# deepaksatna/Distributed-LLM-Training-Benchmark-Framework

Hardware: AMD Instinct MI355X
Metric: tokens_per_sec (higher is better)
Workload: dtype bf16

## Files before the change

### csrc/attention.hip

```cpp
#include <cstdlib>

#ifndef DLTB_ATTN_LPT
#define DLTB_ATTN_LPT 1
#endif
#ifndef DLTB_FWD_KS64
#define DLTB_FWD_KS64 4
#endif
#ifndef DLTB_CAUSAL_KS_CAP
#define DLTB_CAUSAL_KS_CAP 1
#endif
#ifndef DLTB_DQ_KS64
#define DLTB_DQ_KS64 3
#endif
#include "attn_mask.h"
#include "common.h"
#include "mfma_tiles.h"

namespace {

constexpr float kLog2e = 1.4426950408889634f;
constexpr int kBlockRows = 128;
constexpr int kTile = 64;

struct AttnArgs {
// ... 220 lines not shown
}
template <int D>
constexpr int fwd_stage_bytes() { return 2 * kTile * D * 2 + 1024; }
template <int D, int KS = fwd_ks<D>()>
constexpr int fwd_smem_bytes() { return fwd_nst<D, KS>() * KS * fwd_stage_bytes<D>(); }

template <int D, bool CAUSAL, bool DROP, int KS, bool WIN = false, bool DOC = false, bool QR = false>
__global__ __launch_bounds__(256 * KS) void attn_fwd_kernel(AttnArgs P) {
  static_assert(CAUSAL || !WIN, "a window is a band under the causal diagonal");
  static_assert((CAUSAL && !DROP) || !QR, "a query range is causal and without dropout (the packed mask is square)");
  static_assert((CAUSAL && !WIN) || !DOC, "document bounds are causal and carry the window themselves");
  constexpr bool BAND = WIN || DOC;
  constexpr int TB = kTile * D * 2;
  constexpr int NACC = D / 32;
  extern __shared__ __attribute__((aligned(16))) char smem[];
  const int tid = threadIdx.x, lane = tid & 63, w = tid >> 6, r = lane & 31, h = lane >> 5;
  const int qw = w & 3, sp = w >> 2, stid = tid & 255;
  const int T = P.T, nT = T / kTile;
  const int Tq = QR ? P.q_rows : T, qoff = QR ? P.q_begin : 0;
  int qb, bh;
  block_coords(Tq / kBlockRows, P.B * P.Hq, CAUSAL, qb, bh);
  if (QR) qb += qoff / kBlockRows;
  const int b = bh / P.Hq, hq = bh % P.Hq, hk = hq / (P.Hq / P.Hkv);
  const int q0 = qb * kBlockRows + qw * 32;
  const int qi = q0 + r;
  DLTB_DCHECK(qi < T && bh < P.B * P.Hq && hk < P.Hkv);

  bfx8 qf[D / 16];
  {
    const bf16_t* qrow = P.q + ((long)b * Tq + qi - qoff) * P.q_stride + hq * D;
#pragma unroll
    for (int s = 0; s < D / 16; ++s)
      qf[s] = scale_frag(__builtin_bit_cast(bfx8, ld16<uint4>(qrow + 16 * s + 8 * h)), P.scale * kLog2e);
  }
  const int nt = CAUSAL ? min(nT, (qb * kBlockRows + kBlockRows - 1) / kTile + 1) : nT;
  const int W = WIN ? P.window : 0;
  const int lo_q = DOC ? P.bounds[(long)b * T + qi] : 0;
  const int lo_w0 = DOC ? __builtin_amdgcn_readfirstlane(lo_q) : 0;
  const int lo_w1 = DOC ? __builtin_amdgcn_readlane(lo_q, 31) : 0;
  const int t_lo = WIN   ? max(0, qb * kBlockRows - W + 1) / kTile
                   : DOC ? min(max(P.bounds[(long)b * T + qb * kBlockRows], 0), qb * kBlockRows) / kTile
                         : 0;
  const int nit = (nt - t_lo + KS - 1) / KS;
  const bf16_t* kbase = P.k + (long)b * T * P.k_stride + hk * D;
  const bf16_t* vbase = P.v + (long)b * T * P.v_stride + hk * D;
  const uint32_t* mbase = DROP ? P.mask + (long)bh * nT * 2 * T : nullptr;
  const uint32_t* mrow = DROP ? mbase + (long)h * T + qi : nullptr;

  constexpr int NST = fwd_nst<D, KS>();
  constexpr int SB = fwd_stage_bytes<D>();
  constexpr int GL = 2 * GldsTile<D, kTile>::NI + (DROP ? 1 : 0);
  const int wv = __builtin_amdgcn_readfirstlane(qw);
  const int spu = __builtin_amdgcn_readfirstlane(sp);
  auto stage_ptr = [&](int it) { return smem + ((it % NST) * KS + spu) * SB; };
  uint32_t koff[GldsTile<D, kTile>::NI], voff[GldsTile<D, kTile>::NI];
  GldsTile<D, kTile>::offsets(P.k_stride, wv, lane, koff);
  GldsTile<D, kTile>::offsets(P.v_stride, wv, lane, voff);
  const uint32_t moff = (uint32_t)(mrow - mbase) * 4u;
  auto issue = [&](int it) {
    const int t = t_lo + it * KS + spu;
    if (it >= nit || t >= nt) return;
    char* st = smem + ((it % NST) * KS + spu) * SB;
    GldsTile<D, kTile>::load_sv(kbase + (long)t * kTile * P.k_stride, koff, st, wv);
    GldsTile<D, kTile>::load_sv(vbase + (long)t * kTile * P.v_stride, voff, st + TB, wv);
    if (DROP) glds4_sv(mbase + (long)t * 2 * T, moff, st + 2 * TB + wv * 256);
  };
  uint32_t kfo[D / 16], vfo[NACC][2];
#pragma unroll
  for (int s = 0; s < D / 16; ++s) kfo[s] = row_lane_off<D>(r, 2 * s + h);
#pragma unroll
  for (int dt = 0; dt < NACC; ++dt)
#pragma unroll
    for (int hf = 0; hf < 2; ++hf) vfo[dt][hf] = tr_lane_off<D>(dt * 32, hf, lane);
  wait_vm<0>();
#pragma unroll
  for (int i = 0; i < NST - 1; ++i) issue(i);

  f32x16 oacc[NACC];
#pragma unroll
  for (int dt = 0; dt < NACC; ++dt) oacc[dt] = f32x16{};
  float m = -INFINITY, l = 0.f;
  f32x16 mv = f32x16{};
  bool fresh = true;

  f32x16 sacc[2];
  auto s_tile = [&](const char* kt, int kv0) {
    const uint32_t kb = __builtin_amdgcn_readfirstlane(lds_addr(kt));
    uint32_t ka[D / 16];
#pragma unroll
    for (int s = 0; s < D / 16; ++s) ka[s] = lane_addr(kb, kfo[s]);
    sacc[0] = mfma32(row_frag_at<0>(ka[0]), qf[0], mv);
    sacc[1] = mfma32(row_frag_at<32 * D * 2>(ka[0]), qf[0], mv);
    static_for<D / 16 - 1>([&](auto S1) {
      constexpr int s = S1 + 1;
      sacc[0] = mfma32(row_frag_at<0>(ka[s]), qf[s], sacc[0]);
      sacc[1] = mfma32(row_frag_at<32 * D * 2>(ka[s]), qf[s], sacc[1]);
    });
    if (CAUSAL && kv0 + kTile - 1 > q0) {
#pragma unroll
      for (int n = 0; n < 2; ++n)
#pragma unroll
        for (int i = 0; i < 16; ++i)
          if (kv0 + 32 * n + (i & 3) + 8 * (i >> 2) + 4 * h > qi) sacc[n][i] = -INFINITY;
    }
    if (WIN && kv0 <= q0 + 31 - W) {
#pragma unroll
      for (int n = 0; n < 2; ++n)
#pragma unroll
        for (int i = 0; i < 16; ++i)
          if (kv0 + 32 * n + (i & 3) + 8 * (i >> 2) + 4 * h <= qi - W) sacc[n][i] = -INFINITY;
    }
    if (DOC && kv0 < lo_w1) {
#pragma unroll
      for (int n = 0; n < 2; ++n)
#pragma unroll
        for (int i = 0; i < 16; ++i)
          if (kv0 + 32 * n + (i & 3) + 8 * (i >> 2) + 4 * h < lo_q) sacc[n][i] = -INFINITY;
    }
  };
  auto row_max = [&]() {
    float mx = sacc[0][0];
#pragma unroll
    for (int n = 0; n < 2; ++n)
#pragma unroll
      for (int i = (n == 0 ? 1 : 0); i < 16; ++i) mx = fmaxf(mx, sacc[n][i]);
    const auto sw = __builtin_amdgcn_permlane32_swap(__float_as_uint(mx), __float_as_uint(mx), false, false);
    return fmaxf(__uint_as_float(sw[0]), __uint_as_float(sw[1]));
  };
  auto rescale = [&](float mx) {
    const float d = fresh ? mx : fmaxf(mx, 0.f);
    if (!fresh) {
      const float alpha = __builtin_amdgcn_exp2f(-d);
      l *= alpha;
#pragma unroll
      for (int dt = 0; dt < NACC; ++dt) oacc[dt] *= alpha;
    }
    m = fresh ? mx : m + d;
#pragma unroll
    for (int n = 0; n < 2; ++n) sacc[n] -= d;
    mv = splat16(-m);
    fresh = false;
  };
  auto rescale_win = [&](float mx) {
    const bool empty = m == -INFINITY;
    const bool moves = empty ? mx > -INFINITY : mx > kRescaleLog2;
    const float d = moves ? mx : 0.f;
    const float alpha = empty ? 1.f : __builtin_amdgcn_exp2f(-d);
    l *= alpha;
#pragma unroll
    for (int dt = 0; dt < NACC; ++dt) oacc[dt] *= alpha;
    m = moves ? (empty ? mx : m + d) : m;
#pragma unroll
    for (int n = 0; n < 2; ++n) sacc[n] -= d;
    mv = splat16(m == -INFINITY ? 0.f : -m);
  };
  auto softmax = [&]() {
    {
      const float mx = row_max();
      if constexpr (BAND) {
        if (__ballot(m == -INFINITY ? mx > -INFINITY : mx > kRescaleLog2)) rescale_win(mx);
      } else {
        if (fresh || __ballot(mx > kRescaleLog2)) rescale(mx);
      }
    }
    float ls0 = 0.f, ls1 = 0.f;
    static_for<32>([&](auto J) {
      constexpr int n = J / 16, i = J % 16;
      const float p = __builtin_amdgcn_exp2f(sacc[n][i]);
      if constexpr (i & 1) ls1 += p;
      else ls0 += p;
      sacc[n][i] = p;
    });
    l += ls0 + ls1;
  };
  auto pv = [&](const char* vt, uint32_t mw) {
    const uint32_t vb = __builtin_amdgcn_readfirstlane(lds_addr(vt));
    uint32_t va[NACC][2];
#pragma unroll
    for (int dt = 0; dt < NACC; ++dt)
#pragma unroll
      for (int hf = 0; hf < 2; ++hf) va[dt][hf] = lane_addr(vb, vfo[dt][hf]);
    static_for<4>([&](auto J) {
      constexpr int n = J / 2, s2 = J % 2;
      const bfx8 pf = pack_frag_keep<n, s2, DROP>(sacc[n], mw);
#pragma unroll
      for (int dt = 0; dt < NACC; ++dt)
        oacc[dt] = mfma32(tr_frag_at<(32 * n + 16 * s2) * D * 2>(va[dt][0], va[dt][1]), pf, oacc[dt]);
    });
  };
  auto mask_word = [&](const char* st) {
    return DROP ? *reinterpret_cast<const uint32_t*>(st + 2 * TB + wv * 256 + lane * 4) : 0u;
  };
  auto visible = [&](int t) {
    return t < nt && (!CAUSAL || t * kTile <= q0 + 31) && (!WIN || t * kTile + kTile - 1 > q0 - W) &&
           (!DOC || t * kTile + kTile - 1 >= lo_w0);
  };

  {
    for (int it = 0; it < nit; ++it) {
      const int t = t_lo + it * KS + spu;
      static_assert(NST <= 4, "the counted wait below assumes at most two later stages in flight");
      const int later = NST < 3 ? 0 : min(NST - 2, min(nit - 1, (nt - t_lo - 1 - spu) / KS) - it);
      if (NST > 3 && later >= 2) wait_vm<(NST > 3 ? 2 * GL : 0)>();
      else if (NST > 2 && later >= 1) wait_vm<(NST > 2 ? GL : 0)>();
      else wait_vm<0>();
      __builtin_amdgcn_s_barrier();
      issue(it + NST - 1);
      const char* kt = stage_ptr(it);
      if (visible(t)) {
        const uint32_t mw = mask_word(kt);
        s_tile(kt, t * kTile);
        softmax();
        pv(kt + TB, mw);
      }
    }
  }
  __syncthreads();
  if constexpr (KS > 1) {
    constexpr int NF = 16 * NACC + 2;
    static_assert((KS - 1) * 4 * NF * 64 * 4 <= NST * KS * SB, "merge buffer exceeds the LDS ring");
    float* red0 = reinterpret_cast<float*>(smem) + qw * NF * 64 + lane;
    if (sp > 0) {
      float* red = red0 + (sp - 1) * 4 * NF * 64;
      red[0] = m;
      red[64] = l;
#pragma unroll
      for (int dt = 0; dt < NACC; ++dt)
#pragma unroll
        for (int i = 0; i < 16; ++i) red[(2 + 16 * dt + i) * 64] = oacc[dt][i];
    }
    __syncthreads();
    if (sp > 0) return;
#pragma unroll
    for (int o = 0; o < KS - 1; ++o) {
      const float* red = red0 + o * 4 * NF * 64;
      const float m1 = red[0], l1 = red[64];
      const float mn = fmaxf(m, m1);
      const float a0 = BAND && m == -INFINITY ? 0.f : __builtin_amdgcn_exp2f(m - mn);
      const float a1 = BAND && m1 == -INFINITY ? 0.f : __builtin_amdgcn_exp2f(m1 - mn);
      m = mn;
      l = l * a0 + l1 * a1;
#pragma unroll
      for (int dt = 0; dt < NACC; ++dt)
#pragma unroll
        for (int i = 0; i < 16; ++i) oacc[dt][i] = oacc[dt][i] * a0 + red[(2 + 16 * dt + i) * 64] * a1;
    }
  }
  l += __shfl_xor(l, 32, 64);
  const float inv = (DROP ? P.drop_scale : 1.f) / l;
  bf16_t* orow = P.out + ((long)b * Tq + qi - qoff) * P.out_stride + hq * D;
  store_acc_rows<D>(orow, oacc, inv, h);
  if (h == 0) P.lse[((long)b * P.Hq + hq) * Tq + qi - qoff] = (m + __log2f(l)) * 0.69314718055994531f;
}



template <int D>
__global__ __launch_bounds__(256) void attn_bwd_delta_kernel(AttnArgs P) {
  constexpr int CH = D / 8;
  const long gid = blockIdx.x * (long)blockDim.x + threadIdx.x;
  const long row = gid / CH;
// ... 384 lines not shown
    const bf16_t* dorow = P.dout + ((long)b * Tq + qi - qoff) * P.do_stride + hq * D;
#pragma unroll
    for (int s = 0; s < D / 16; ++s) {
      qf[s] = __builtin_bit_cast(bfx8, ld16<uint4>(qrow + 16 * s + 8 * h));
      of[s] = __builtin_bit_cast(bfx8, ld16<uint4>(dorow + 16 * s + 8 * h));
    }
  }
  float dlt;
  if (P.o) {
    const bf16_t* orow = P.o + ((long)b * Tq + qi - qoff) * P.o_stride + hq * D;
    constexpr int NS = D / 16;
    float cs[NS];
#pragma unroll
    for (int s = 0; s < NS; ++s) {
      float a[8], c[8];
      unpack8(ld16<uint4>(orow + 16 * s + 8 * h), a);
      unpack8(__builtin_bit_cast(uint4, of[s]), c);
      float acc = 0.f;
#pragma unroll
      for (int e = 0; e < 8; ++e) acc += c[e] * a[e];
      cs[s] = acc;
    }
#pragma unroll
    for (int off = NS / 2; off > 0; off >>= 1)
#pragma unroll
      for (int s = 0; s < off; ++s) cs[s] += cs[s + off];
    dlt = cs[0] + __shfl_xor(cs[0], 32, 64);
    if (sp == 0 && h == 0) const_cast<float*>(P.delta)[bq * Tq + qi - qoff] = dlt;
  } else {
    dlt = P.delta[bq * Tq + qi - qoff];
  }
  const f32x16 nlv = splat16(-P.lse[bq * Tq + qi - qoff] * kLog2e);
  const float nd = -dlt * (DROP ? 1.f / P.drop_scale : 1.f);
  const f32x16 ndv = splat16(nd);
#pragma unroll
  for (int s = 0; s < D / 16; ++s) qf[s] = scale_frag(qf[s], P.scale * kLog2e);
  const uint32_t* mbase = DROP ? P.mask + (long)bq * nT * 2 * T : nullptr;
  const uint32_t* mrow = DROP ? mbase + (long)h * T + qi : nullptr;
  const int nt = CAUSAL ? min(nT, (qb * kBlockRows + kBlockRows - 1) / kTile + 1) : nT;
  const int W = WIN ? P.window : 0;
  const int lo_q = DOC ? P.bounds[(long)b * T + qi] : 0;
  const int lo_w0 = DOC ? __builtin_amdgcn_readfirstlane(lo_q) : 0;
  const int lo_w1 = DOC ? __builtin_amdgcn_readlane(lo_q, 31) : 0;
  const int t_lo = WIN   ? max(0, qb * kBlockRows - W + 1) / kTile
                   : DOC ? min(max(P.bounds[(long)b * T + qb * kBlockRows], 0), qb * kBlockRows) / kTile
                         : 0;
  const int nit = (nt - t_lo + KS - 1) / KS;
  const bf16_t* kbase = P.k + (long)b * T * P.k_stride + hk * D;
  const bf16_t* vbase = P.v + (long)b * T * P.v_stride + hk * D;

  constexpr int NST = dq_nst<D>();
  constexpr int SB = dq_stage_bytes<D>();
  constexpr int GL = 2 * GldsTile<D, kTile>::NI + (DROP ? 1 : 0);
  const int wv = __builtin_amdgcn_readfirstlane(qw);
  auto stage_ptr = [&](int it) { return smem + ((it % NST) * KS + sp) * SB; };
  uint32_t koff[GldsTile<D, kTile>::NI], voff[GldsTile<D, kTile>::NI];
  GldsTile<D, kTile>::offsets(P.k_stride, wv, lane, koff);
  GldsTile<D, kTile>::offsets(P.v_stride, wv, lane, voff);
  const uint32_t moff = (uint32_t)(mrow - mbase) * 4u;
  const int spu = __builtin_amdgcn_readfirstlane(sp);
  auto issue = [&](int it) {
    const int t = t_lo + it * KS + spu;
    if (it >= nit || t >= nt) return;
    char* st = smem + ((it % NST) * KS + spu) * SB;
    GldsTile<D, kTile>::load_sv(kbase + (long)t * kTile * P.k_stride, koff, st, wv);
    GldsTile<D, kTile>::load_sv(vbase + (long)t * kTile * P.v_stride, voff, st + TB, wv);
    if (DROP) glds4_sv(mbase + (long)t * 2 * T, moff, st + 2 * TB + wv * 256);
  };
  wait_vm<0>();
#pragma unroll
  for (int i = 0; i < NST - 1; ++i) issue(i);

  constexpr bool EMU2 = DOC && D == 128 && DROP && KS == 1;
  f32x16 dq[NACC], dq_odd[EMU2 ? NACC : 1];
#pragma unroll
  for (int dt = 0; dt < NACC; ++dt) dq[dt] = f32x16{};
  if constexpr (EMU2) {
#pragma unroll
    for (int dt = 0; dt < NACC; ++dt) dq_odd[dt] = f32x16{};
  }

  for (int it = 0; it < nit; ++it) {
    const int t = t_lo + it * KS + sp;
    static_assert(NST <= 3, "the counted wait below assumes at most one later stage in flight");
    if (NST > 2 && it + 1 < nit && t_lo + (it + 1) * KS + sp < nt) wait_vm<(NST > 2 ? GL : 0)>();
    else wait_vm<0>();
    __builtin_amdgcn_s_barrier();
    issue(it + NST - 1);
    const char* kt = stage_ptr(it);
    const char* vt = kt + TB;
    const uint32_t mw = DROP ? *reinterpret_cast<const uint32_t*>(kt + 2 * TB + wv * 256 + lane * 4) : 0u;
    const int kv0 = t * kTile;
    auto sdp = [&](int n, f32x16& sa, f32x16& dp) {
      sa = nlv;
      dp = ndv;
#pragma unroll
      for (int s = 0; s < D / 16; ++s) {
        sa = mfma32(row_frag<D>(kt, 32 * n + r, 2 * s + h), qf[s], sa);
        dp = mfma32(row_frag<D>(vt, 32 * n + r, 2 * s + h), of[s], dp);
      }
    };
    auto fin = [&](int n, const f32x16& sa, const f32x16& dp, auto ODD) {
      const bool diag = CAUSAL && kv0 + 32 * n + 31 > q0;
      const bool ledge = WIN && kv0 + 32 * n <= q0 + 31 - W;
      const bool dedge = DOC && kv0 + 32 * n < lo_w1;
      f32x16 ds;
      static_for<16>([&](auto I) {
        constexpr int i = I;
        float p = __builtin_amdgcn_exp2f(sa[i]);
        if (diag && kv0 + 32 * n + (i & 3) + 8 * (i >> 2) + 4 * h > qi) p = 0.f;
        if (ledge && kv0 + 32 * n + (i & 3) + 8 * (i >> 2) + 4 * h <= qi - W) p = 0.f;
        if (dedge && kv0 + 32 * n + (i & 3) + 8 * (i >> 2) + 4 * h < lo_q) p = 0.f;
        const float dpv = DROP ? (n == 0 ? keep_sel<mask_bit(0, i)>(dp[i], nd, mw)
                                         : keep_sel<mask_bit(1, i)>(dp[i], nd, mw)) : dp[i];
        ds[i] = p * dpv;
      });
#pragma unroll
      for (int s2 = 0; s2 < 2; ++s2) {
        const bfx8 sf = pack_frag<D>(ds, s2);
#pragma unroll
        for (int dt = 0; dt < NACC; ++dt)
          if constexpr (EMU2 && ODD) dq_odd[dt] = mfma32(tr_frag<D>(kt, 32 * n + 16 * s2, dt * 32, lane), sf, dq_odd[dt]);
          else dq[dt] = mfma32(tr_frag<D>(kt, 32 * n + 16 * s2, dt * 32, lane), sf, dq[dt]);
      }
    };
    if (t < nt) {
      {
#pragma unroll
        for (int n = 0; n < 2; ++n) {
          if (CAUSAL && kv0 + 32 * n > q0 + 31) continue;
          if (WIN && kv0 + 32 * n + 31 <= q0 - W) continue;
          if (DOC && kv0 + 32 * n + 31 < lo_w0) continue;
          f32x16 sa, dp;
          sdp(n, sa, dp);
          if (EMU2 && (it & 1)) fin(n, sa, dp, IC<1>{});
          else fin(n, sa, dp, IC<0>{});
        }
      }
    }
  }
  if constexpr (EMU2) {
#pragma unroll
    for (int dt = 0; dt < NACC; ++dt)
#pragma unroll
      for (int i = 0; i < 16; ++i) dq[dt][i] += dq_odd[dt][i];
  }
  __syncthreads();
  if constexpr (KS > 1) {
    constexpr int NF = 16 * NACC;
    static_assert((KS - 1) * 4 * NF * 64 * 4 <= dq_smem_bytes<D, KS>(), "merge buffer exceeds the LDS ring");
    float* red0 = reinterpret_cast<float*>(smem) + qw * NF * 64 + lane;
    if (sp > 0) {
      float* red = red0 + (sp - 1) * 4 * NF * 64;
#pragma unroll
      for (int dt = 0; dt < NACC; ++dt)
#pragma unroll
        for (int i = 0; i < 16; ++i) red[(16 * dt + i) * 64] = dq[dt][i];
    }
    __syncthreads();
    if (sp > 0) return;
#pragma unroll
    for (int o = 0; o < KS - 1; ++o)
#pragma unroll
      for (int dt = 0; dt < NACC; ++dt)
#pragma unroll
        for (int i = 0; i < 16; ++i) dq[dt][i] += red0[o * 4 * NF * 64 + (16 * dt + i) * 64];
  }
  bf16_t* dqrow = P.out + ((long)b * Tq + qi - qoff) * P.out_stride + hq * D;
  store_acc_rows<D>(dqrow, dq, P.scale * (DROP ? P.drop_scale : 1.f), h);
}

AttnArgs make_args(const void* q, const void* k, const void* v, long qs, long ks, long vs, int B,
                   int T, int Hq, int Hkv, float scale, int causal, uint32_t thr16,
                   float drop_scale, const int64_t* seed, int64_t site) {
  AttnArgs a{};
  a.q = (const bf16_t*)q;
  a.k = (const bf16_t*)k;
  a.v = (const bf16_t*)v;
  a.q_stride = qs;
  a.k_stride = ks;
  a.v_stride = vs;
  a.B = B;
  a.T = T;
  a.Hq = Hq;
  a.Hkv = Hkv;
  a.scale = scale;
  a.causal = causal;
  a.thr16 = thr16;
  a.drop_scale = drop_scale;
// ... 40 lines not shown
}

template <int D, bool C, bool DR, bool WIN = false, bool DOC = false, bool QR = false>
void launch_fwd(const AttnArgs& a, hipStream_t st) {
  constexpr int KS = fwd_ks<D, C>();
  constexpr int smem = fwd_smem_bytes<D, KS>();
  dim3 grid(((QR ? a.q_rows : a.T) / kBlockRows) * a.B * a.Hq);
  hipLaunchKernelGGL((attn_fwd_kernel<D, C, DR, KS, WIN, DOC, QR>), grid, dim3(256 * KS), smem, st, a);
}

#define DLTB_ATTN_DISPATCH(FN, D, C, DR, ...)           \
  do {                                                  \
    if (D == 64) {                                      \
      if (C) { if (DR) FN<64, true, true>(__VA_ARGS__); else FN<64, true, false>(__VA_ARGS__); } \
      else   { if (DR) FN<64, false, true>(__VA_ARGS__); else FN<64, false, false>(__VA_ARGS__); } \
    } else {                                            \
      if (C) { if (DR) FN<128, true, true>(__VA_ARGS__); else FN<128, true, false>(__VA_ARGS__); } \
      else   { if (DR) FN<128, false, true>(__VA_ARGS__); else FN<128, false, false>(__VA_ARGS__); } \
    }                                                   \
  } while (0)

#define DLTB_ATTN_DISPATCH_WIN(FN, D, DR, ...)          \
  do {                                                  \
    if (D == 64) { if (DR) FN<64, true, true, true>(__VA_ARGS__); else FN<64, true, false, true>(__VA_ARGS__); } \
    else         { if (DR) FN<128, true, true, true>(__VA_ARGS__); else FN<128, true, false, true>(__VA_ARGS__); } \
  } while (0)

#define DLTB_ATTN_DISPATCH_DOC(FN, D, DR, ...)          \
  do {                                                  \
    if (D == 64) { if (DR) FN<64, true, true, false, true>(__VA_ARGS__); else FN<64, true, false, false, true>(__VA_ARGS__); } \
    else         { if (DR) FN<128, true, true, false, true>(__VA_ARGS__); else FN<128, true, false, false, true>(__VA_ARGS__); } \
  } while (0)

#define DLTB_ATTN_DISPATCH_QR(FN, D, WIN, DOC, ...)     \
  do {                                                  \
    if (D == 64) {                                      \
      if (DOC) FN<64, true, false, false, true, true>(__VA_ARGS__);         \
      else if (WIN) FN<64, true, false, true, false, true>(__VA_ARGS__);    \
      else FN<64, true, false, false, false, true>(__VA_ARGS__);            \
    } else {                                            \
      if (DOC) FN<128, true, false, false, true, true>(__VA_ARGS__);        \
      else if (WIN) FN<128, true, false, true, false, true>(__VA_ARGS__);   \
      else FN<128, true, false, false, false, true>(__VA_ARGS__);           \
    }                                                   \
  } while (0)

bool windowed(int causal, int window, int T) { return causal && window > 0 && window < T; }

bool ranged(int q_begin, int q_end, int T) { return q_end > 0 && !(q_begin == 0 && q_end == T); }

}

void dltb_attn_init_attributes() {
  static bool done = false;
  if (done) return;
  done = true;
  set_attrs<64, false, false>();
  set_attrs<64, false, true>();
  set_attrs<64, true, false>();
  set_attrs<64, true, true>();
  set_attrs<128, false, false>();
  set_attrs<128, false, true>();
  set_attrs<128, true, false>();
  set_attrs<128, true, true>();
  set_attrs<64, true, false, true>();
  set_attrs<64, true, true, true>();
  set_attrs<128, true, false, true>();
  set_attrs<128, true, true, true>();
  set_attrs<64, true, false, false, true>();
  set_attrs<64, true, true, false, true>();
  set_attrs<128, true, false, false, true>();
  set_attrs<128, true, true, false, true>();
  set_attrs_qr<64, false, false>();
  set_attrs_qr<64, true, false>();
  set_attrs_qr<64, false, true>();
  set_attrs_qr<128, false, false>();
  set_attrs_qr<128, true, false>();
  set_attrs_qr<128, false, true>();
}

void dltb_attn_doc_bounds(const int64_t* idx, int* bounds, int B, int T, int64_t eos, int window, hipStream_t st) {
  hipLaunchKernelGGL(attn_doc_bounds_kernel, dim3(B), dim3(256), 0, st, idx, bounds, B, T, eos,
                     window > 0 && window < T ? window : 0);
}

void dltb_attn_mask(uint32_t* mask, int B, int T, int Hq, uint32_t thr16, const int64_t* seed,
                    int64_t site, hipStream_t st) {
  const dim3 grid(cdiv(T, 256), (unsigned)(B * Hq * (T / kTile) * 2));
  hipLaunchKernelGGL(attn_mask_kernel, grid, dim3(256), 0, st, mask, T, thr16, seed, site);
}

void dltb_attn_fwd(const void* q, const void* k, const void* v, void* o, float* lse,
                   const uint32_t* mask, long qs, long ks, long vs, long os, int B, int T, int Hq,
                   int Hkv, int D, float scale, int causal, uint32_t thr16, float drop_scale,
                   hipStream_t st, int window, const int* bounds, int q_begin, int q_end) {
  AttnArgs a = make_args(q, k, v, qs, ks, vs, B, T, Hq, Hkv, scale, causal, thr16, drop_scale,
                         nullptr, 0);
  a.out = (bf16_t*)o;
  a.out_stride = os;
  a.lse = lse;
  a.mask = mask;
  if (ranged(q_begin, q_end, T)) {
    a.q_begin = q_begin;
    a.q_rows = q_end - q_begin;
    a.bounds = bounds;
    a.window = windowed(causal, window, T) ? window : 0;
    DLTB_ATTN_DISPATCH_QR(launch_fwd, D, a.window != 0, bounds != nullptr, a, st);
    return;
  }
// ... 132 lines not shown
```

### csrc/gemm_tn.hip

```cpp
#include "common.h"
#include "launchers.h"
#include "mfma_tiles.h"

namespace {

constexpr int kTM = 256, kTN = 256;
constexpr int kRowB = 512;

struct TnArgs {
  const bf16_t* a;
  const bf16_t* b;
  bf16_t* c;
  long lda, ldb, ldc;
  long sa, sb, sc;
  int M, N, K, batch;
  int accumulate;
};

typedef __attribute__((ext_vector_type(4))) float f4;

DLTB_DEV f4 mfma16(bfx8 a, bfx8 b, f4 c) {
#if DLTB_F16
  return __builtin_amdgcn_mfma_f32_16x16x32_f16(a, b, c, 0, 0, 0);
#else
// ... 136 lines not shown
    o.y = pack_bf2(v[2], v[3]);
    *reinterpret_cast<uint2*>(cbase + (long)(16 * i) * g.ldc + 16 * j) = o;
  };
  if (g.accumulate) {
    uint2 old[8][4];
#pragma unroll
    for (int i = 0; i < 8; ++i)
#pragma unroll
      for (int j = 0; j < 4; ++j) old[i][j] = *reinterpret_cast<const uint2*>(cbase + (long)(16 * i) * g.ldc + 16 * j);
#pragma unroll
    for (int i = 0; i < 8; ++i)
#pragma unroll
      for (int j = 0; j < 4; ++j) {
        const float v[4] = {acc[i][j][0] + lo_bf(old[i][j].x), acc[i][j][1] + hi_bf(old[i][j].x),
                            acc[i][j][2] + lo_bf(old[i][j].y), acc[i][j][3] + hi_bf(old[i][j].y)};
        store(i, j, v);
      }
  } else {
#pragma unroll
    for (int i = 0; i < 8; ++i)
#pragma unroll
      for (int j = 0; j < 4; ++j) {
        const float v[4] = {acc[i][j][0], acc[i][j][1], acc[i][j][2], acc[i][j][3]};
        store(i, j, v);
      }
  }
}

}

bool dltb_gemm_tn_supported(int M, int N, int K) {
  return M > 0 && N > 0 && K > 0 && M % kTM == 0 && N % kTN == 0 && K % (2 * kTK3) == 0 && K / kTK3 >= 4;
}

int dltb_gemm_tn(const void* a, const void* b, void* c, long lda, long ldb, long ldc, long sa, long sb, long sc,
                 int M, int N, int K, int batch, int accumulate, hipStream_t st) {
  if (!dltb_gemm_tn_supported(M, N, K) || batch < 1) return -1;
  TnArgs g{};
  g.a = (const bf16_t*)a;
  g.b = (const bf16_t*)b;
  g.c = (bf16_t*)c;
  g.lda = lda;
  g.ldb = ldb;
  g.ldc = ldc;
  g.sa = sa;
  g.sb = sb;
  g.sc = sc;
  g.M = M;
  g.N = N;
  g.K = K;
  g.batch = batch;
  g.accumulate = accumulate;
  constexpr int smem = kRing3 * kStage3;
  static bool attr = false;
  if (!attr) {
    (void)hipFuncSetAttribute((const void*)gemm_tn_kernel, hipFuncAttributeMaxDynamicSharedMemorySize, smem);
    attr = true;
  }
  const dim3 grid((unsigned)((long)(M / kTM) * (N / kTN) * batch));
  hipLaunchKernelGGL(gemm_tn_kernel, grid, dim3(512), smem, st, g);
  return 0;
}
```

### csrc/mfma_tiles.h

```cpp
#pragma once
#include "common.h"

namespace {

typedef h16_t bfx8 __attribute__((ext_vector_type(8)));
typedef short s16x4 __attribute__((ext_vector_type(4)));
typedef __attribute__((address_space(3))) s16x4 lds_s16x4;

DLTB_DEV f32x16 mfma32(bfx8 a, bfx8 b, f32x16 c) {
#if DLTB_F16
  return __builtin_amdgcn_mfma_f32_32x32x16_f16(a, b, c, 0, 0, 0);
#else
  return __builtin_amdgcn_mfma_f32_32x32x16_bf16(a, b, c, 0, 0, 0);
#endif
}

template <int D>
DLTB_DEV int swz(int row) {
  if constexpr (D == 32) return (row >> 2) & 3;
  if constexpr (D == 64) return (((row >> 1) & 1) << 2) | ((row >> 2) & 3);
  else return ((row & 3) << 2) | ((row >> 2) & 3);
}
template <int D>
DLTB_DEV int toff(int row, int ch) {
  return row * (D * 2) + ((ch ^ swz<D>(row)) << 4);
}

template <int D>
DLTB_DEV bfx8 row_frag(const char* tile, int row, int ch) {
  uint4 v = *reinterpret_cast<const uint4*>(tile + toff<D>(row, ch));
  return __builtin_bit_cast(bfx8, v);
}

template <int D>
DLTB_DEV bfx8 tr_frag(const char* tile, int row_base, int col_base, int lane) {
  const int g = lane >> 4, i = lane & 15;
  const int row = row_base + 4 * (g >> 1) + (i >> 2);
  const int col = col_base + 16 * (g & 1) + 4 * (i & 3);
  const char* p0 = tile + toff<D>(row, col >> 3) + (col & 7) * 2;
  const char* p1 = tile + toff<D>(row + 8, col >> 3) + (col & 7) * 2;
  s16x4 a = __builtin_amdgcn_ds_read_tr16_b64_v4i16((lds_s16x4*)p0);
  s16x4 b = __builtin_amdgcn_ds_read_tr16_b64_v4i16((lds_s16x4*)p1);
  typedef short s16x8 __attribute__((ext_vector_type(8)));
  s16x8 c = {a[0], a[1], a[2], a[3], b[0], b[1], b[2], b[3]};
  return __builtin_bit_cast(bfx8, c);
}

template <int D>
DLTB_DEV uint32_t row_lane_off(int lane_row, int ch) { return (uint32_t)toff<D>(lane_row, ch); }
template <int D>
DLTB_DEV uint32_t tr_lane_off(int col_base, int half, int lane) {
  const int g = lane >> 4, i = lane & 15;
  const int row = 4 * (g >> 1) + (i >> 2) + 8 * half;
  const int col = col_base + 16 * (g & 1) + 4 * (i & 3);
  return (uint32_t)(toff<D>(row, col >> 3) + (col & 7) * 2);
}
typedef __attribute__((address_space(3))) const char lds_cchar;
typedef __attribute__((address_space(3))) const uint4 lds_u4;
DLTB_DEV uint32_t lds_addr(const void* p) { return (uint32_t)(size_t)(lds_cchar*)p; }
DLTB_DEV uint32_t lane_addr(uint32_t sbase, uint32_t off) {
  uint32_t a;
  asm("v_add_u32 %0, %1, %2" : "=v"(a) : "s"(sbase), "v"(off));
  return a;
}
template <int OFF>
DLTB_DEV bfx8 row_frag_at(uint32_t a) { return __builtin_bit_cast(bfx8, *(lds_u4*)(size_t)(a + OFF)); }
template <int OFF>
DLTB_DEV bfx8 tr_frag_at(uint32_t a0, uint32_t a1) {
  s16x4 a = __builtin_amdgcn_ds_read_tr16_b64_v4i16((lds_s16x4*)(size_t)(a0 + OFF));
  s16x4 b = __builtin_amdgcn_ds_read_tr16_b64_v4i16((lds_s16x4*)(size_t)(a1 + OFF));
  typedef short s16x8 __attribute__((ext_vector_type(8)));
  s16x8 c = {a[0], a[1], a[2], a[3], b[0], b[1], b[2], b[3]};
  return __builtin_bit_cast(bfx8, c);
}

DLTB_DEV void glds16_asm(const void* gsrc, const void* lds_dst) {
  const uint32_t lds = __builtin_amdgcn_readfirstlane(
      (uint32_t)(uintptr_t)(const __attribute__((address_space(3))) char*)lds_dst);
  uint32_t keep;
  asm volatile("s_mov_b32 %0, m0\n\ts_mov_b32 m0, %2\n\ts_nop 0\n\tglobal_load_lds_dwordx4 %1, off\n\ts_mov_b32 m0, %0"
               : "=&s"(keep)
               : "v"(gsrc), "s"(lds)
               : "memory");
}

DLTB_DEV void glds4_asm(const void* gsrc, const void* lds_dst) {
  const uint32_t lds = __builtin_amdgcn_readfirstlane(
      (uint32_t)(uintptr_t)(const __attribute__((address_space(3))) char*)lds_dst);
  uint32_t keep;
  asm volatile("s_mov_b32 %0, m0\n\ts_mov_b32 m0, %2\n\ts_nop 0\n\tglobal_load_lds_dword %1, off\n\ts_mov_b32 m0, %0"
               : "=&s"(keep)
               : "v"(gsrc), "s"(lds)
               : "memory");
}

DLTB_DEV uint64_t uniform_ptr(const void* p) {
  const uint64_t b = (uint64_t)(uintptr_t)p;
  const uint32_t hi = (uint32_t)__builtin_amdgcn_readfirstlane((uint32_t)(b >> 32));
  const uint32_t lo = (uint32_t)__builtin_amdgcn_readfirstlane((uint32_t)b);
  return ((uint64_t)hi << 32) | (uint64_t)lo;
}
DLTB_DEV void glds16_sv(const void* sbase, uint32_t voff, const void* lds_dst) {
  const uint32_t lds = __builtin_amdgcn_readfirstlane(
      (uint32_t)(uintptr_t)(const __attribute__((address_space(3))) char*)lds_dst);
  uint32_t keep;
  asm volatile("s_mov_b32 %0, m0\n\ts_mov_b32 m0, %3\n\ts_nop 0\n\tglobal_load_lds_dwordx4 %1, %2\n\ts_mov_b32 m0, %0"
               : "=&s"(keep)
               : "v"(voff), "s"(uniform_ptr(sbase)), "s"(lds)
               : "memory");
}
DLTB_DEV void glds4_sv(const void* sbase, uint32_t voff, const void* lds_dst) {
  const uint32_t lds = __builtin_amdgcn_readfirstlane(
      (uint32_t)(uintptr_t)(const __attribute__((address_space(3))) char*)lds_dst);
  uint32_t keep;
  asm volatile("s_mov_b32 %0, m0\n\ts_mov_b32 m0, %3\n\ts_nop 0\n\tglobal_load_lds_dword %1, %2\n\ts_mov_b32 m0, %0"
               : "=&s"(keep)
               : "v"(voff), "s"(uniform_ptr(sbase)), "s"(lds)
               : "memory");
}

template <int N>
DLTB_DEV void wait_vm() {
  static_assert(N >= 0 && N < 64, "vmcnt range");
  __builtin_amdgcn_s_waitcnt((N & 15) | ((N >> 4) << 14) | (7 << 4) | (15 << 8));
}

DLTB_DEV int swap23(int r) { return (r & ~12) | ((r & 4) << 1) | ((r & 8) >> 1); }

template <int D, int ROWS, bool ASM = false, bool KSWAP = false>
struct GldsTile {
  static constexpr int CH = D / 8;
  static constexpr int NI = ROWS * CH / 256;
  static_assert(ROWS * CH % 256 == 0, "tile must split into whole wave-instructions");
  static_assert(!KSWAP || ROWS % 16 == 0, "swap23 permutes rows within aligned groups of 16");
  DLTB_DEV static void load(const bf16_t* base, long stride, int row0, char* tile, int wv, int lane) {
#pragma unroll
    for (int i = 0; i < NI; ++i) {
      const int lin = (wv * NI + i) * 64 + lane;
      const int row = lin / CH, pos = lin % CH;
      const int srow = KSWAP ? swap23(row) : row;
      const bf16_t* src = base + (long)(row0 + srow) * stride + ((pos ^ swz<D>(row)) << 3);
      if constexpr (ASM)
        glds16_asm(src, tile + (wv * NI + i) * 1024);
      else
        __builtin_amdgcn_global_load_lds((const void*)src,
                                         (__attribute__((address_space(3))) void*)(tile + (wv * NI + i) * 1024),
                                         16, 0, 0);
    }
  }
  DLTB_DEV static void offsets(long stride, int wv, int lane, uint32_t (&off)[NI]) {
    static_assert(!KSWAP, "the hoisted-offset form has no row permutation");
#pragma unroll
    for (int i = 0; i < NI; ++i) {
      const int lin = (wv * NI + i) * 64 + lane;
      const int row = lin / CH, pos = lin % CH;
      off[i] = (uint32_t)((row * stride + ((pos ^ swz<D>(row)) << 3)) * 2);
    }
  }
  DLTB_DEV static void load_sv(const bf16_t* base_row0, const uint32_t (&off)[NI], char* tile, int wv) {
#pragma unroll
    for (int i = 0; i < NI; ++i) glds16_sv(base_row0, off[i], tile + (wv * NI + i) * 1024);
  }
};

}
```

Measured before the change: 294,800.

## Fuse stage loads into one asm block with incrementing scalar pointers and ring slots

Replaces the per-tile global-to-LDS load lambdas in the forward attention kernel with one inline-asm routine that issues all K, V and mask pieces while setting M0 once per piece. Scalar base pointers and LDS ring offsets now advance incrementally, so the per-iteration modulo and 64-bit address math go away. A specialised non-causal D=64 dQ backward loop uses the same scheme with precomputed LDS lane addresses. It also tracks per-device attribute initialisation. The changes cut scalar and vector address overhead in the pipelined load loop, but they limit the forward path to at most three stages (NST 2 or 3) and lean on hand-written asm.

```diff
diff --git a/csrc/attention.hip b/csrc/attention.hip
--- a/csrc/attention.hip
+++ b/csrc/attention.hip
@@ -296,18 +296,27 @@
   constexpr int GL = 2 * GldsTile<D, kTile>::NI + (DROP ? 1 : 0);
   const int wv = __builtin_amdgcn_readfirstlane(qw);
   const int spu = __builtin_amdgcn_readfirstlane(sp);
-  auto stage_ptr = [&](int it) { return smem + ((it % NST) * KS + spu) * SB; };
   uint32_t koff[GldsTile<D, kTile>::NI], voff[GldsTile<D, kTile>::NI];
   GldsTile<D, kTile>::offsets(P.k_stride, wv, lane, koff);
   GldsTile<D, kTile>::offsets(P.v_stride, wv, lane, voff);
   const uint32_t moff = (uint32_t)(mrow - mbase) * 4u;
-  auto issue = [&](int it) {
-    const int t = t_lo + it * KS + spu;
-    if (it >= nit || t >= nt) return;
-    char* st = smem + ((it % NST) * KS + spu) * SB;
-    GldsTile<D, kTile>::load_sv(kbase + (long)t * kTile * P.k_stride, koff, st, wv);
-    GldsTile<D, kTile>::load_sv(vbase + (long)t * kTile * P.v_stride, voff, st + TB, wv);
-    if (DROP) glds4_sv(mbase + (long)t * 2 * T, moff, st + 2 * TB + wv * 256);
+  const int n_my = (nt - t_lo - spu + KS - 1) / KS;
+  const uint32_t lds0 = __builtin_amdgcn_readfirstlane(lds_addr(smem)) + (uint32_t)(spu * SB);
+  const uint32_t ldsk = lds0 + (uint32_t)(wv * GldsTile<D, kTile>::NI * 1024), ldsm = lds0 + 2 * TB + (uint32_t)(wv * 256);
+  const long tf = t_lo + spu;
+  uint64_t kp = uniform_ptr(kbase + tf * kTile * P.k_stride), vp = uniform_ptr(vbase + tf * kTile * P.v_stride);
+  uint64_t mp = DROP ? uniform_ptr(mbase + tf * 2 * T) : 0;
+  const uint64_t kstep = (uint64_t)(KS * kTile * 2) * (uint64_t)P.k_stride;
+  const uint64_t vstep = (uint64_t)(KS * kTile * 2) * (uint64_t)P.v_stride, mstep = (uint64_t)(KS * 2 * 4) * (uint64_t)T;
+  constexpr uint32_t kSlot = KS * SB, kRingEnd = (NST - 1) * KS * SB;
+  uint32_t wslot = 0, rslot = 0;
+  auto issue = [&](int i) {
+    if (i >= n_my) return;
+    glds_stage<GldsTile<D, kTile>::NI, TB, DROP>(kp, koff, vp, voff, mp, moff, ldsk + wslot, ldsm + wslot);
+    kp += kstep;
+    vp += vstep;
+    if (DROP) mp += mstep;
+    wslot = wslot == kRingEnd ? 0u : wslot + kSlot;
   };
   uint32_t kfo[D / 16], vfo[NACC][2];
 #pragma unroll
@@ -328,8 +337,7 @@
   bool fresh = true;
 
   f32x16 sacc[2];
-  auto s_tile = [&](const char* kt, int kv0) {
-    const uint32_t kb = __builtin_amdgcn_readfirstlane(lds_addr(kt));
+  auto s_tile = [&](uint32_t kb, int kv0) {
     uint32_t ka[D / 16];
 #pragma unroll
     for (int s = 0; s < D / 16; ++s) ka[s] = lane_addr(kb, kfo[s]);
@@ -417,8 +425,7 @@
     });
     l += ls0 + ls1;
   };
-  auto pv = [&](const char* vt, uint32_t mw) {
-    const uint32_t vb = __builtin_amdgcn_readfirstlane(lds_addr(vt));
+  auto pv = [&](uint32_t vb, uint32_t mw) {
     uint32_t va[NACC][2];
 #pragma unroll
     for (int dt = 0; dt < NACC; ++dt)
@@ -432,25 +439,23 @@
         oacc[dt] = mfma32(tr_frag_at<(32 * n + 16 * s2) * D * 2>(va[dt][0], va[dt][1]), pf, oacc[dt]);
     });
   };
-  auto mask_word = [&](const char* st) {
-    return DROP ? *reinterpret_cast<const uint32_t*>(st + 2 * TB + wv * 256 + lane * 4) : 0u;
-  };
+  const uint32_t mwo = (uint32_t)(2 * TB + wv * 256 + lane * 4);
+  auto mask_word = [&](uint32_t st) { return DROP ? lds_ld32(st + mwo) : 0u; };
   auto visible = [&](int t) {
     return t < nt && (!CAUSAL || t * kTile <= q0 + 31) && (!WIN || t * kTile + kTile - 1 > q0 - W) &&
            (!DOC || t * kTile + kTile - 1 >= lo_w0);
   };
 
   {
-    for (int it = 0; it < nit; ++it) {
-      const int t = t_lo + it * KS + spu;
-      static_assert(NST <= 4, "the counted wait below assumes at most two later stages in flight");
-      const int later = NST < 3 ? 0 : min(NST - 2, min(nit - 1, (nt - t_lo - 1 - spu) / KS) - it);
-      if (NST > 3 && later >= 2) wait_vm<(NST > 3 ? 2 * GL : 0)>();
-      else if (NST > 2 && later >= 1) wait_vm<(NST > 2 ? GL : 0)>();
+    static_assert(NST == 2 || NST == 3, "the counted wait below assumes at most one later stage in flight");
+    int t = t_lo + spu;
+    for (int it = 0; it < nit; ++it, t += KS) {
+      if (NST > 2 && it + 1 < n_my) wait_vm<(NST > 2 ? GL : 0)>();
       else wait_vm<0>();
       __builtin_amdgcn_s_barrier();
       issue(it + NST - 1);
-      const char* kt = stage_ptr(it);
+      const uint32_t kt = lds0 + rslot;
+      rslot = rslot == kRingEnd ? 0u : rslot + kSlot;
       if (visible(t)) {
         const uint32_t mw = mask_word(kt);
         s_tile(kt, t * kTile);
@@ -941,25 +946,6 @@
   constexpr int NST = dq_nst<D>();
   constexpr int SB = dq_stage_bytes<D>();
   constexpr int GL = 2 * GldsTile<D, kTile>::NI + (DROP ? 1 : 0);
-  const int wv = __builtin_amdgcn_readfirstlane(qw);
-  auto stage_ptr = [&](int it) { return smem + ((it % NST) * KS + sp) * SB; };
-  uint32_t koff[GldsTile<D, kTile>::NI], voff[GldsTile<D, kTile>::NI];
-  GldsTile<D, kTile>::offsets(P.k_stride, wv, lane, koff);
-  GldsTile<D, kTile>::offsets(P.v_stride, wv, lane, voff);
-  const uint32_t moff = (uint32_t)(mrow - mbase) * 4u;
-  const int spu = __builtin_amdgcn_readfirstlane(sp);
-  auto issue = [&](int it) {
-    const int t = t_lo + it * KS + spu;
-    if (it >= nit || t >= nt) return;
-    char* st = smem + ((it % NST) * KS + spu) * SB;
-    GldsTile<D, kTile>::load_sv(kbase + (long)t * kTile * P.k_stride, koff, st, wv);
-    GldsTile<D, kTile>::load_sv(vbase + (long)t * kTile * P.v_stride, voff, st + TB, wv);
-    if (DROP) glds4_sv(mbase + (long)t * 2 * T, moff, st + 2 * TB + wv * 256);
-  };
-  wait_vm<0>();
-#pragma unroll
-  for (int i = 0; i < NST - 1; ++i) issue(i);
-
   constexpr bool EMU2 = DOC && D == 128 && DROP && KS == 1;
   f32x16 dq[NACC], dq_odd[EMU2 ? NACC : 1];
 #pragma unroll
@@ -969,61 +955,161 @@
     for (int dt = 0; dt < NACC; ++dt) dq_odd[dt] = f32x16{};
   }
 
-  for (int it = 0; it < nit; ++it) {
-    const int t = t_lo + it * KS + sp;
-    static_assert(NST <= 3, "the counted wait below assumes at most one later stage in flight");
-    if (NST > 2 && it + 1 < nit && t_lo + (it + 1) * KS + sp < nt) wait_vm<(NST > 2 ? GL : 0)>();
-    else wait_vm<0>();
-    __builtin_amdgcn_s_barrier();
-    issue(it + NST - 1);
-    const char* kt = stage_ptr(it);
-    const char* vt = kt + TB;
-    const uint32_t mw = DROP ? *reinterpret_cast<const uint32_t*>(kt + 2 * TB + wv * 256 + lane * 4) : 0u;
-    const int kv0 = t * kTile;
-    auto sdp = [&](int n, f32x16& sa, f32x16& dp) {
-      sa = nlv;
-      dp = ndv;
-#pragma unroll
-      for (int s = 0; s < D / 16; ++s) {
-        sa = mfma32(row_frag<D>(kt, 32 * n + r, 2 * s + h), qf[s], sa);
-        dp = mfma32(row_frag<D>(vt, 32 * n + r, 2 * s + h), of[s], dp);
-      }
+  constexpr bool DIET = D == 64 && !CAUSAL;
+  if constexpr (DIET) {
+    const int wv = __builtin_amdgcn_readfirstlane(qw);
+    const int spu = __builtin_amdgcn_readfirstlane(sp);
+    uint32_t koff[GldsTile<D, kTile>::NI], voff[GldsTile<D, kTile>::NI];
+    GldsTile<D, kTile>::offsets(P.k_stride, wv, lane, koff);
+    GldsTile<D, kTile>::offsets(P.v_stride, wv, lane, voff);
+    const uint32_t moff = (uint32_t)(mrow - mbase) * 4u;
+    const int n_my = (nt - t_lo - spu + KS - 1) / KS;
+    const uint32_t lds0 = __builtin_amdgcn_readfirstlane(lds_addr(smem)) + (uint32_t)(spu * SB);
+    const uint32_t ldsk = lds0 + (uint32_t)(wv * GldsTile<D, kTile>::NI * 1024), ldsm = lds0 + 2 * TB + (uint32_t)(wv * 256);
+    const long tf = t_lo + spu;
+    uint64_t kp = uniform_ptr(kbase + tf * kTile * P.k_stride), vp = uniform_ptr(vbase + tf * kTile * P.v_stride);
+    uint64_t mp = DROP ? uniform_ptr(mbase + tf * 2 * T) : 0;
+    const uint64_t kstep = (uint64_t)(KS * kTile * 2) * (uint64_t)P.k_stride;
+    const uint64_t vstep = (uint64_t)(KS * kTile * 2) * (uint64_t)P.v_stride, mstep = (uint64_t)(KS * 2 * 4) * (uint64_t)T;
+    constexpr uint32_t kSlot = KS * SB, kRingEnd = (NST - 1) * KS * SB;
+    uint32_t wslot = 0, rslot = 0;
+    auto issue = [&](int i) {
+      if (i >= n_my) return;
+      glds_stage<GldsTile<D, kTile>::NI, TB, DROP>(kp, koff, vp, voff, mp, moff, ldsk + wslot, ldsm + wslot);
+      kp += kstep;
+      vp += vstep;
+      if (DROP) mp += mstep;
+      wslot = wslot == kRingEnd ? 0u : wslot + kSlot;
     };
-    auto fin = [&](int n, const f32x16& sa, const f32x16& dp, auto ODD) {
-      const bool diag = CAUSAL && kv0 + 32 * n + 31 > q0;
-      const bool ledge = WIN && kv0 + 32 * n <= q0 + 31 - W;
-      const bool dedge = DOC && kv0 + 32 * n < lo_w1;
-      f32x16 ds;
-      static_for<16>([&](auto I) {
-        constexpr int i = I;
-        float p = __builtin_amdgcn_exp2f(sa[i]);
-        if (diag && kv0 + 32 * n + (i & 3) + 8 * (i >> 2) + 4 * h > qi) p = 0.f;
-        if (ledge && kv0 + 32 * n + (i & 3) + 8 * (i >> 2) + 4 * h <= qi - W) p = 0.f;
-        if (dedge && kv0 + 32 * n + (i & 3) + 8 * (i >> 2) + 4 * h < lo_q) p = 0.f;
-        const float dpv = DROP ? (n == 0 ? keep_sel<mask_bit(0, i)>(dp[i], nd, mw)
-                                         : keep_sel<mask_bit(1, i)>(dp[i], nd, mw)) : dp[i];
-        ds[i] = p * dpv;
+    wait_vm<0>();
+#pragma unroll
+    for (int i = 0; i < NST - 1; ++i) issue(i);
+
+    static_assert(NST == 2 || NST == 3, "the counted wait below assumes at most one later stage in flight");
+    static_assert(!CAUSAL && !WIN && !DOC && !EMU2, "this loop has no mask and one accumulator set");
+    const uint32_t mwo = (uint32_t)(2 * TB + wv * 256 + lane * 4);
+    uint32_t kfo[D / 16], tfo[NACC][2];
+#pragma unroll
+    for (int s = 0; s < D / 16; ++s) kfo[s] = row_lane_off<D>(r, 2 * s + h);
+#pragma unroll
+    for (int dt = 0; dt < NACC; ++dt)
+#pragma unroll
+      for (int hf = 0; hf < 2; ++hf) tfo[dt][hf] = tr_lane_off<D>(dt * 32, hf, lane);
+    for (int it = 0; it < nit; ++it) {
+      if (NST > 2 && it + 1 < n_my) wait_vm<(NST > 2 ? GL : 0)>();
+      else wait_vm<0>();
+      __builtin_amdgcn_s_barrier();
+      issue(it + NST - 1);
+      const uint32_t kt = lds0 + rslot;
+      rslot = rslot == kRingEnd ? 0u : rslot + kSlot;
+      if (it >= n_my) continue;
+      const uint32_t mw = DROP ? lds_ld32(kt + mwo) : 0u;
+      uint32_t ka[D / 16], ta[NACC][2];
+#pragma unroll
+      for (int s = 0; s < D / 16; ++s) ka[s] = lane_addr(kt, kfo[s]);
+#pragma unroll
+      for (int dt = 0; dt < NACC; ++dt)
+#pragma unroll
+        for (int hf = 0; hf < 2; ++hf) ta[dt][hf] = lane_addr(kt, tfo[dt][hf]);
+      static_for<2>([&](auto N) {
+        constexpr int n = N;
+        f32x16 sa = nlv, dp = ndv, ds;
+        static_for<D / 16>([&](auto S) {
+          constexpr int s = S;
+          sa = mfma32(row_frag_at<32 * n * D * 2>(ka[s]), qf[s], sa);
+          dp = mfma32(row_frag_at<TB + 32 * n * D * 2>(ka[s]), of[s], dp);
+        });
+        static_for<16>([&](auto I) {
+          constexpr int i = I;
+          const float p = __builtin_amdgcn_exp2f(sa[i]);
+          const float dpv = DROP ? keep_sel<mask_bit(n, i)>(dp[i], nd, mw) : dp[i];
+          ds[i] = p * dpv;
+        });
+        static_for<2>([&](auto S2) {
+          constexpr int s2 = S2;
+          const bfx8 sf = pack_frag<D>(ds, s2);
+#pragma unroll
+          for (int dt = 0; dt < NACC; ++dt)
+            dq[dt] = mfma32(tr_frag_at<(32 * n + 16 * s2) * D * 2>(ta[dt][0], ta[dt][1]), sf, dq[dt]);
+        });
       });
-#pragma unroll
-      for (int s2 = 0; s2 < 2; ++s2) {
-        const bfx8 sf = pack_frag<D>(ds, s2);
-#pragma unroll
-        for (int dt = 0; dt < NACC; ++dt)
-          if constexpr (EMU2 && ODD) dq_odd[dt] = mfma32(tr_frag<D>(kt, 32 * n + 16 * s2, dt * 32, lane), sf, dq_odd[dt]);
-          else dq[dt] = mfma32(tr_frag<D>(kt, 32 * n + 16 * s2, dt * 32, lane), sf, dq[dt]);
-      }
+    }
+  } else {
+    const int wv = __builtin_amdgcn_readfirstlane(qw);
+    auto stage_ptr = [&](int it) { return smem + ((it % NST) * KS + sp) * SB; };
+    uint32_t koff[GldsTile<D, kTile>::NI], voff[GldsTile<D, kTile>::NI];
+    GldsTile<D, kTile>::offsets(P.k_stride, wv, lane, koff);
+    GldsTile<D, kTile>::offsets(P.v_stride, wv, lane, voff);
+    const uint32_t moff = (uint32_t)(mrow - mbase) * 4u;
+    const int spu = __builtin_amdgcn_readfirstlane(sp);
+    auto issue = [&](int it) {
+      const int t = t_lo + it * KS + spu;
+      if (it >= nit || t >= nt) return;
+      char* st = smem + ((it % NST) * KS + spu) * SB;
+      GldsTile<D, kTile>::load_sv(kbase + (long)t * kTile * P.k_stride, koff, st, wv);
+      GldsTile<D, kTile>::load_sv(vbase + (long)t * kTile * P.v_stride, voff, st + TB, wv);
+      if (DROP) glds4_sv(mbase + (long)t * 2 * T, moff, st + 2 * TB + wv * 256);
     };
-    if (t < nt) {
-      {
-#pragma unroll
-        for (int n = 0; n < 2; ++n) {
-          if (CAUSAL && kv0 + 32 * n > q0 + 31) continue;
-          if (WIN && kv0 + 32 * n + 31 <= q0 - W) continue;
-          if (DOC && kv0 + 32 * n + 31 < lo_w0) continue;
-          f32x16 sa, dp;
-          sdp(n, sa, dp);
-          if (EMU2 && (it & 1)) fin(n, sa, dp, IC<1>{});
-          else fin(n, sa, dp, IC<0>{});
+    wait_vm<0>();
+#pragma unroll
+    for (int i = 0; i < NST - 1; ++i) issue(i);
+
+    for (int it = 0; it < nit; ++it) {
+      const int t = t_lo + it * KS + sp;
+      static_assert(NST <= 3, "the counted wait below assumes at most one later stage in flight");
+      if (NST > 2 && it + 1 < nit && t_lo + (it + 1) * KS + sp < nt) wait_vm<(NST > 2 ? GL : 0)>();
+      else wait_vm<0>();
+      __builtin_amdgcn_s_barrier();
+      issue(it + NST - 1);
+      const char* kt = stage_ptr(it);
+      const char* vt = kt + TB;
+      const uint32_t mw = DROP ? *reinterpret_cast<const uint32_t*>(kt + 2 * TB + wv * 256 + lane * 4) : 0u;
+      const int kv0 = t * kTile;
+      auto sdp = [&](int n, f32x16& sa, f32x16& dp) {
+        sa = nlv;
+        dp = ndv;
+#pragma unroll
+        for (int s = 0; s < D / 16; ++s) {
+          sa = mfma32(row_frag<D>(kt, 32 * n + r, 2 * s + h), qf[s], sa);
+          dp = mfma32(row_frag<D>(vt, 32 * n + r, 2 * s + h), of[s], dp);
+        }
+      };
+      auto fin = [&](int n, const f32x16& sa, const f32x16& dp, auto ODD) {
+        const bool diag = CAUSAL && kv0 + 32 * n + 31 > q0;
+        const bool ledge = WIN && kv0 + 32 * n <= q0 + 31 - W;
+        const bool dedge = DOC && kv0 + 32 * n < lo_w1;
+        f32x16 ds;
+        static_for<16>([&](auto I) {
+          constexpr int i = I;
+          float p = __builtin_amdgcn_exp2f(sa[i]);
+          if (diag && kv0 + 32 * n + (i & 3) + 8 * (i >> 2) + 4 * h > qi) p = 0.f;
+          if (ledge && kv0 + 32 * n + (i & 3) + 8 * (i >> 2) + 4 * h <= qi - W) p = 0.f;
+          if (dedge && kv0 + 32 * n + (i & 3) + 8 * (i >> 2) + 4 * h < lo_q) p = 0.f;
+          const float dpv = DROP ? (n == 0 ? keep_sel<mask_bit(0, i)>(dp[i], nd, mw)
+                                           : keep_sel<mask_bit(1, i)>(dp[i], nd, mw)) : dp[i];
+          ds[i] = p * dpv;
+        });
+#pragma unroll
+        for (int s2 = 0; s2 < 2; ++s2) {
+          const bfx8 sf = pack_frag<D>(ds, s2);
+#pragma unroll
+          for (int dt = 0; dt < NACC; ++dt)
+            if constexpr (EMU2 && ODD) dq_odd[dt] = mfma32(tr_frag<D>(kt, 32 * n + 16 * s2, dt * 32, lane), sf, dq_odd[dt]);
+            else dq[dt] = mfma32(tr_frag<D>(kt, 32 * n + 16 * s2, dt * 32, lane), sf, dq[dt]);
+        }
+      };
+      if (t < nt) {
+        {
+#pragma unroll
+          for (int n = 0; n < 2; ++n) {
+            if (CAUSAL && kv0 + 32 * n > q0 + 31) continue;
+            if (WIN && kv0 + 32 * n + 31 <= q0 - W) continue;
+            if (DOC && kv0 + 32 * n + 31 < lo_w0) continue;
+            f32x16 sa, dp;
+            sdp(n, sa, dp);
+            if (EMU2 && (it & 1)) fin(n, sa, dp, IC<1>{});
+            else fin(n, sa, dp, IC<0>{});
+          }
         }
       }
     }
@@ -1170,9 +1256,13 @@
 }
 
 void dltb_attn_init_attributes() {
-  static bool done = false;
-  if (done) return;
-  done = true;
+  static bool done[64] = {};
+  int dev = 0;
+  (void)hipGetDevice(&dev);
+  if (dev >= 0 && dev < 64) {
+    if (done[dev]) return;
+    done[dev] = true;
+  }
   set_attrs<64, false, false>();
   set_attrs<64, false, true>();
   set_attrs<64, true, false>();
diff --git a/csrc/gemm_tn.hip b/csrc/gemm_tn.hip
--- a/csrc/gemm_tn.hip
+++ b/csrc/gemm_tn.hip
@@ -212,10 +212,12 @@
   g.batch = batch;
   g.accumulate = accumulate;
   constexpr int smem = kRing3 * kStage3;
-  static bool attr = false;
-  if (!attr) {
+  static bool attr[64] = {};
+  int dev = 0;
+  (void)hipGetDevice(&dev);
+  if (dev < 0 || dev >= 64 || !attr[dev]) {
     (void)hipFuncSetAttribute((const void*)gemm_tn_kernel, hipFuncAttributeMaxDynamicSharedMemorySize, smem);
-    attr = true;
+    if (dev >= 0 && dev < 64) attr[dev] = true;
   }
   const dim3 grid((unsigned)((long)(M / kTM) * (N / kTN) * batch));
   hipLaunchKernelGGL(gemm_tn_kernel, grid, dim3(512), smem, st, g);
diff --git a/csrc/mfma_tiles.h b/csrc/mfma_tiles.h
--- a/csrc/mfma_tiles.h
+++ b/csrc/mfma_tiles.h
@@ -46,6 +46,25 @@
   return __builtin_bit_cast(bfx8, c);
 }
 
+typedef __attribute__((address_space(3))) const uint4 lds_cu4;
+template <int D>
+DLTB_DEV bfx8 row_frag_a(uint32_t tile, int row, int ch) {
+  return __builtin_bit_cast(bfx8, *(lds_cu4*)(size_t)(tile + (uint32_t)toff<D>(row, ch)));
+}
+template <int D>
+DLTB_DEV bfx8 tr_frag_a(uint32_t tile, int row_base, int col_base, int lane) {
+  const int g = lane >> 4, i = lane & 15;
+  const int row = row_base + 4 * (g >> 1) + (i >> 2);
+  const int col = col_base + 16 * (g & 1) + 4 * (i & 3);
+  const uint32_t p0 = tile + (uint32_t)(toff<D>(row, col >> 3) + (col & 7) * 2);
+  const uint32_t p1 = tile + (uint32_t)(toff<D>(row + 8, col >> 3) + (col & 7) * 2);
+  s16x4 a = __builtin_amdgcn_ds_read_tr16_b64_v4i16((lds_s16x4*)(size_t)p0);
+  s16x4 b = __builtin_amdgcn_ds_read_tr16_b64_v4i16((lds_s16x4*)(size_t)p1);
+  typedef short s16x8 __attribute__((ext_vector_type(8)));
+  s16x8 c = {a[0], a[1], a[2], a[3], b[0], b[1], b[2], b[3]};
+  return __builtin_bit_cast(bfx8, c);
+}
+
 template <int D>
 DLTB_DEV uint32_t row_lane_off(int lane_row, int ch) { return (uint32_t)toff<D>(lane_row, ch); }
 template <int D>
@@ -117,6 +136,61 @@
                : "=&s"(keep)
                : "v"(voff), "s"(uniform_ptr(sbase)), "s"(lds)
                : "memory");
+}
+
+#define DLTB_GLDS_HEAD "s_mov_b32 %[keep], m0\n\ts_mov_b32 m0, %[lds]\n\ts_nop 0\n\tglobal_load_lds_dwordx4 %[a0], %[pa]\n\t"
+#define DLTB_GLDS_PIECE(OFF, V, P) \
+  "s_add_u32 m0, %[lds], %[" #OFF "]\n\ts_nop 0\n\tglobal_load_lds_dwordx4 %[" #V "], %[" #P "]\n\t"
+#define DLTB_GLDS_WORD "s_mov_b32 m0, %[ldsw]\n\ts_nop 0\n\tglobal_load_lds_dword %[w], %[pw]\n\t"
+#define DLTB_GLDS_TAIL "s_mov_b32 m0, %[keep]"
+template <int NI, int TB, bool WORD>
+DLTB_DEV void glds_stage(uint64_t pa, const uint32_t (&oa)[NI], uint64_t pb, const uint32_t (&ob)[NI], uint64_t pw,
+                         uint32_t ow, uint32_t lds, uint32_t ldsw) {
+  static_assert(NI == 2 || NI == 4, "two or four 1 KiB pieces per wave and image");
+  uint32_t keep;
+  if constexpr (NI == 2 && WORD) {
+    asm volatile(DLTB_GLDS_HEAD DLTB_GLDS_PIECE(i1, a1, pa) DLTB_GLDS_PIECE(j0, b0, pb) DLTB_GLDS_PIECE(j1, b1, pb)
+                     DLTB_GLDS_WORD DLTB_GLDS_TAIL
+                 : [keep] "=&s"(keep)
+                 : [a0] "v"(oa[0]), [a1] "v"(oa[1]), [b0] "v"(ob[0]), [b1] "v"(ob[1]), [w] "v"(ow), [pa] "s"(pa),
+                   [pb] "s"(pb), [pw] "s"(pw), [lds] "s"(lds), [ldsw] "s"(ldsw), [i1] "n"(1024), [j0] "n"(TB),
+                   [j1] "n"(TB + 1024)
+                 : "memory", "scc");
+  } else if constexpr (NI == 2) {
+    asm volatile(DLTB_GLDS_HEAD DLTB_GLDS_PIECE(i1, a1, pa) DLTB_GLDS_PIECE(j0, b0, pb) DLTB_GLDS_PIECE(j1, b1, pb)
+                     DLTB_GLDS_TAIL
+                 : [keep] "=&s"(keep)
+                 : [a0] "v"(oa[0]), [a1] "v"(oa[1]), [b0] "v"(ob[0]), [b1] "v"(ob[1]), [pa] "s"(pa), [pb] "s"(pb),
+                   [lds] "s"(lds), [i1] "n"(1024), [j0] "n"(TB), [j1] "n"(TB + 1024)
+                 : "memory", "scc");
+  } else if constexpr (WORD) {
+    asm volatile(DLTB_GLDS_HEAD DLTB_GLDS_PIECE(i1, a1, pa) DLTB_GLDS_PIECE(i2, a2, pa) DLTB_GLDS_PIECE(i3, a3, pa)
+                     DLTB_GLDS_PIECE(j0, b0, pb) DLTB_GLDS_PIECE(j1, b1, pb) DLTB_GLDS_PIECE(j2, b2, pb)
+                         DLTB_GLDS_PIECE(j3, b3, pb) DLTB_GLDS_WORD DLTB_GLDS_TAIL
+                 : [keep] "=&s"(keep)
+                 : [a0] "v"(oa[0]), [a1] "v"(oa[1]), [a2] "v"(oa[2]), [a3] "v"(oa[3]), [b0] "v"(ob[0]), [b1] "v"(ob[1]),
+                   [b2] "v"(ob[2]), [b3] "v"(ob[3]), [w] "v"(ow), [pa] "s"(pa), [pb] "s"(pb), [pw] "s"(pw),
+                   [lds] "s"(lds), [ldsw] "s"(ldsw), [i1] "n"(1024), [i2] "n"(2048), [i3] "n"(3072), [j0] "n"(TB),
+                   [j1] "n"(TB + 1024), [j2] "n"(TB + 2048), [j3] "n"(TB + 3072)
+                 : "memory", "scc");
+  } else {
+    asm volatile(DLTB_GLDS_HEAD DLTB_GLDS_PIECE(i1, a1, pa) DLTB_GLDS_PIECE(i2, a2, pa) DLTB_GLDS_PIECE(i3, a3, pa)
+                     DLTB_GLDS_PIECE(j0, b0, pb) DLTB_GLDS_PIECE(j1, b1, pb) DLTB_GLDS_PIECE(j2, b2, pb)
+                         DLTB_GLDS_PIECE(j3, b3, pb) DLTB_GLDS_TAIL
+                 : [keep] "=&s"(keep)
+                 : [a0] "v"(oa[0]), [a1] "v"(oa[1]), [a2] "v"(oa[2]), [a3] "v"(oa[3]), [b0] "v"(ob[0]), [b1] "v"(ob[1]),
+                   [b2] "v"(ob[2]), [b3] "v"(ob[3]), [pa] "s"(pa), [pb] "s"(pb), [lds] "s"(lds), [i1] "n"(1024),
+                   [i2] "n"(2048), [i3] "n"(3072), [j0] "n"(TB), [j1] "n"(TB + 1024), [j2] "n"(TB + 2048),
+                   [j3] "n"(TB + 3072)
+                 : "memory", "scc");
+  }
+}
+#undef DLTB_GLDS_HEAD
+#undef DLTB_GLDS_PIECE
+#undef DLTB_GLDS_WORD
+#undef DLTB_GLDS_TAIL
+DLTB_DEV uint32_t lds_ld32(uint32_t a) {
+  return *(const __attribute__((address_space(3))) uint32_t*)(size_t)a;
 }
 
 template <int N>
```

Result: no change. 296,300, median of 6 (+0.5%).
